# google-research/nerf-from-image

Measured on NVIDIA H100. Metric: rays_per_sec_128x128_64+64spp, higher is better.
Workload: dtype f32

## Files before the change

nerf_from_image_b200/csrc/nfi_forward_pipe.cuh:

```cuda
#pragma once
#include <type_traits>

#include "nfi_forward_tc.cuh"

namespace nfi {

#ifndef NFI_WAIT_NS
#define NFI_WAIT_NS 0
#endif
#define NFI_STEP_WAIT(bar, par) tc::mbar_wait_backoff<NFI_WAIT_NS>(bar, par)

__device__ __forceinline__ void mbar_arrive(uint64_t* bar) {
  asm volatile("mbarrier.arrive.shared::cta.b64 _, [%0];" ::"r"(tc::smem_u32(bar)) : "memory");
}

__device__ __forceinline__ float ld_relaxed(const float* p) {
  float v;
  asm volatile("ld.relaxed.cta.global.f32 %0, [%1];" : "=f"(v) : "l"(p) : "memory");
  return v;
}

__device__ __forceinline__ void column_sort(float* col, int n, int stride) {
  const int gaps[4] = {23, 10, 4, 1};
#pragma unroll 1
  for (int gi = 0; gi < 4; ++gi) {
    const int gap = gaps[gi];
    for (int i = gap; i < n; ++i) {
      const float v = col[i * stride];
      int j = i - gap;
      while (j >= 0 && col[j * stride] > v) {
        col[(j + gap) * stride] = col[j * stride];
        j -= gap;
      }
      col[(j + gap) * stride] = v;
    }
  }
}

__device__ __forceinline__ bool elect_one() {
  uint32_t pred;
  asm volatile(
      "{\n.reg .pred p;\nelect.sync _|p, 0xffffffff;\nselp.u32 %0, 1, 0, p;\n}\n"
      : "=r"(pred));
  return pred != 0;
}

struct TileCoord {
  int b, tile_x, tile_y;
};

__device__ __forceinline__ TileCoord tile_coord(int tile, int tiles_x, int tiles_y) {
  TileCoord c;
  const int per_img = tiles_x * tiles_y;
  c.b = tile / per_img;
  const int r = tile % per_img;
  const int bx = (tiles_x + 1) / 2;
  const int blk = r / 4, in = r % 4;
  int tx = 2 * (blk % bx) + (in & 1), ty = 2 * (blk / bx) + (in >> 1);
  if ((tiles_x & 1) || (tiles_y & 1)) {
    tx = r % tiles_x;
    ty = r / tiles_x;
  }
  c.tile_x = tx;
  c.tile_y = ty;
  return c;
}

constexpr int kPipeSlots = 3;
constexpr int kPipeStageBytes = 32768;
constexpr int kFwdStageBytes = 32768;
constexpr int kD2Ld = 20;
constexpr int kD2SlotBytes = kThreads * kD2Ld * 4;

__host__ __device__ inline size_t pipe_scratch_floats(int S, int nes) {
  return tc_scratch_floats_per_group(S) + (size_t)S * kThreads * nes;
}

template <int P>
struct PipeCfg {
  static constexpr int kThreadsTotal = 256 + 128 * P;
  static constexpr int kStages = P + 1;
  static constexpr int kSmA = 25600;
  static constexpr int kSmD2 = kSmA + kStages * kFwdStageBytes;
  static constexpr int kSmPal = kSmD2 + kPipeSlots * kD2SlotBytes;
  static constexpr int kSmFrac = kSmPal + 48 * 4;
  static constexpr int kSmBars = kSmFrac + 128 * 4;
  static constexpr int kNumBars = 2 * kStages + 2 * kPipeSlots + 3;
  static constexpr int kSmBytes = kSmBars + kNumBars * 8;
  static constexpr int kActRegs = 136;
  static constexpr int kShadeRegs = 80;
  static constexpr int kProducerRegs = 88;
};

constexpr float kLog2e = 1.4426950408889634f;
constexpr float kLn2 = 0.6931471805599453f;
constexpr float kPadLogit = -1e30f;

template <typename F>
__device__ __forceinline__ void decoder_step(uint64_t dsc_a, uint64_t w1_hi, uint64_t w1_lo,
                                             uint64_t w2_hi, uint64_t w2_lo,
                                             const float* __restrict__ b1, float* d2, int warp,
                                             int lane, F&& on_stage_read) {
#pragma unroll 1
  for (int mb = 0; mb < 2; ++mb) {
    float d[32];
#pragma unroll
    for (int i = 0; i < 32; ++i) d[i] = 0.f;
    tc::wgmma_fence();
    tc::layer1_mb(d, dsc_a + mb * (8192 >> 4), dsc_a + ((16384 + mb * 8192) >> 4), w1_hi, w1_lo);
    tc::wgmma_commit();
    tc::wgmma_wait<0>();
    tc::reg_fence(d);
    if (mb == 1) on_stage_read();
    uint32_t hi[8][4], lo[8][4];
    tc::softplus_frag<true>(d, b1, lane & 3, hi, lo);
    float o[8];
#pragma unroll
    for (int i = 0; i < 8; ++i) o[i] = 0.f;
    tc::wgmma_fence();
    tc::layer2_mb(o, hi, lo, w2_hi, w2_lo);
    tc::wgmma_commit();
    tc::wgmma_wait<0>();
    tc::reg_fence(o);
    tc::store_frag_rows(o, d2 + 64 * mb * kD2Ld, kD2Ld, warp, lane);
  }
}

__device__ __forceinline__ float ldcg(const float* p) {
  float v;
  asm volatile("ld.global.cg.f32 %0, [%1];" : "=f"(v) : "l"(p));
  return v;
}

template <int NOUT_PAD>
__device__ __forceinline__ void field_head_fast(const float (&out)[NOUT_PAD], const FieldConst& fc,
                                                const float* __restrict__ pal, float keep,
                                                float& sigma, float& cr, float& cg, float& cb,
                                                float* probs = nullptr) {
  constexpr int NA = NOUT_PAD - 1;
  const float d = out[0];
  if (fc.use_sdf) {
    const float nd = -d;
    const float e = tc::ex2_approx(-fabsf(nd) * (fc.inv_beta * kLog2e));
    const float sg = (nd > 0.f) ? 1.f : ((nd < 0.f) ? -1.f : 0.f);
    const float cdf = 0.5f + 0.5f * sg * (1.f - e);
    sigma = fc.inv_alpha * (cdf * keep);
  } else {
    const float x = d - 1.f;
    sigma = (x > 20.f ? x : log1pf(expf(x))) * keep;
  }
  if (fc.A > 0) {
    float m = out[1];
#pragma unroll
    for (int a = 1; a < NA; ++a) m = fmaxf(m, out[1 + a]);
    float pv[((3 * NA + 3) / 4) * 4];
#pragma unroll
    for (int i = 0; i < (3 * NA + 3) / 4; ++i) {
      const float4 t = *reinterpret_cast<const float4*>(pal + 4 * i);
      pv[4 * i] = t.x;
      pv[4 * i + 1] = t.y;
      pv[4 * i + 2] = t.z;
      pv[4 * i + 3] = t.w;
    }
    float s = 0.f, r = 0.f, g = 0.f, b = 0.f;
#pragma unroll
    for (int a = 0; a < NA; ++a) {
      const float e = tc::ex2_approx(out[1 + a] - m);
      if (probs != nullptr) probs[a] = e;
      s += e;
      r = fmaf(e, pv[3 * a + 0], r);
      g = fmaf(e, pv[3 * a + 1], g);
      b = fmaf(e, pv[3 * a + 2], b);
    }
    const float inv = __fdividef(1.f, s);
    cr = r * inv;
    cg = g * inv;
    cb = b * inv;
    if (probs != nullptr) {
#pragma unroll
      for (int a = 0; a < NA; ++a) probs[a] *= inv;
    }
  } else {
    cr = sigmoid_fast(out[1]) * 2.004f - 1.002f;
    cg = sigmoid_fast(out[2]) * 2.004f - 1.002f;
    cb = sigmoid_fast(out[3]) * 2.004f - 1.002f;
  }
}

template <int N>
struct LaneVec {
  float v[N];
};
template <int N>
__device__ __forceinline__ LaneVec<N> shift_down1(const LaneVec<N>& x, float pad, int lane) {
  LaneVec<N> y;
#pragma unroll
  for (int i = 0; i < N; ++i) {
    const float a = __shfl_down_sync(kFull, x.v[i], 1);
    const float nxt0 = (i + 1 < N) ? __shfl_sync(kFull, x.v[(i + 1 < N) ? i + 1 : i], 0) : pad;
    y.v[i] = (lane == 31) ? nxt0 : a;
  }
  return y;
}
template <int N>
__device__ __forceinline__ float pick(const LaneVec<N>& x, int idx) {
  float r = __shfl_sync(kFull, x.v[0], idx & 31);
#pragma unroll
// ... 244 lines not shown

  constexpr int kRsParts = 2 + P;
  auto rs_first = [](int part) {
    constexpr int base_rows = 32 / kRsParts, rem = 32 % kRsParts;
    return part * base_rows + min(max(part - 2, 0), rem);
  };
  auto resample_rows = [&](int part, float tnear, float tfar, size_t ray, bool valid) {
    const int first = rs_first(part), count = rs_first(part + 1) - first;
    ResampleArgs ra;
    ra.sc_w = sc_w;
    ra.sc_zf = sc_zf;
    ra.z_fine = p.z_fine;
    ra.noise_t = p.noise_t;
    ra.noise_u = p.noise_u;
    ra.frac = frac;
    ra.S = S;
    ra.wig = wig;
    ra.explicit_noise = explicit_noise;
    resample_rows_impl<NSLOT>(ra, first, count, tnear, tfar, ray, valid, lane);
  };

  if (wg >= 3) {
    asm volatile("setmaxnreg.dec.sync.aligned.u32 %0;" ::"n"(Cfg::kProducerRegs));
    const int set = wg - 3;
    uint32_t n = 0;
    uint32_t tile_it = 0;
    for (int tile = blockIdx.x; tile < n_tiles; tile += gridDim.x, ++tile_it) {
      const TileCoord tcd = tile_coord(tile, tiles_x, tiles_y);
      const int b = tcd.b;
      int px, py;
      tile_pixel(tcd.tile_x, tcd.tile_y, wig, lane, px, py);
      const bool valid = (px < p.width) && (py < p.height);
      px = min(px, p.width - 1);
      py = min(py, p.height - 1);
      const size_t ray = ((size_t)b * p.height + py) * p.width + px;
      Ray r;
      setup_ray(p, b, py, px, r);
      const float span = r.tfar - r.tnear;
      const uint32_t plane_bytes = (uint32_t)R * (uint32_t)R * 128u;
      const unsigned char* planes_b =
          reinterpret_cast<const unsigned char*>(p.planes) + (size_t)b * 3 * plane_bytes;
      for (int pass = 0; pass < (FINE ? 2 : 1); ++pass) {
        if (pass == 1) {
          tc::mbar_wait(cw_ready, tile_it & 1);
          resample_rows(2 + set, r.tnear, r.tfar, ray, valid);
          __threadfence_block();
          __syncwarp();
          if (lane == 0) mbar_arrive(zf_ready);
          tc::mbar_wait(zf_ready, tile_it & 1);
        }
        int s = (int)(((uint32_t)set + (uint32_t)P - (n % P)) % P);
        auto fetch = [&](int ss) -> float {
          if (ss >= S) return 0.f;
          if (pass == 0) return explicit_noise ? p.noise_t[ray * S + ss] : 0.f;
          return ld_relaxed(sc_zf + ss * kThreads + gt);
        };
        float nxt = fetch(s);
        for (; s < S; s += P) {
          const uint32_t st = (n + (uint32_t)s) % NS, u = (n + (uint32_t)s) / NS;
          unsigned char* const stage = base + Cfg::kSmA + st * kFwdStageBytes;
          const float cur = nxt;
          nxt = fetch(s + P);
          if (DBG && dbg_time) tprev = clock64();
          NFI_STEP_WAIT(&a_free[st], (u & 1) ^ 1);
          NFI_T(0)
          float t;
          if (pass == 0)
            t = lerp_torch(r.tnear, r.tfar, frac[s]) + cur * (span / (float)S);
          else
            t = cur;
          const float x0 = (r.ox + r.dx * t) * inv_range, x1 = (r.oy + r.dy * t) * inv_range,
                      x2 = (r.oz + r.dz * t) * inv_range;
          ByteTaps tp;
          byte_taps(x0, x1, R, 0u, tp.o[0], tp.fx[0], tp.fy[0]);
          byte_taps(x0, x2, R, plane_bytes >> 4, tp.o[1], tp.fx[1], tp.fy[1]);
          byte_taps(x1, x2, R, plane_bytes >> 3, tp.o[2], tp.fx[2], tp.fy[2]);
          NFI_T(1)
          if (dbg_window) {
            tp.o[0] &= 0x7FFu;
            tp.o[1] &= 0x7FFu;
            tp.o[2] &= 0x7FFu;
          }
          if (!dbg_skip_gather)
            gather_to_tiles_lean(planes_b, R, tp, stage, stage + 16384, 32 * wig, lane);
          NFI_T(2)
          tc::fence_async_smem();
          __syncwarp();
          if (lane == 0) mbar_arrive(&full[st]);
          NFI_T(3)
          if (DBG && dbg_time) tacc[9] += 1;
        }
        n += (uint32_t)S;
      }
    }
    if (DBG && dbg_time)
      for (int i = 0; i < 10; ++i) p.normals[i] = (float)tacc[i];
  } else if (wg == 0) {
    asm volatile("setmaxnreg.inc.sync.aligned.u32 %0;" ::"n"(Cfg::kActRegs));
    const uint32_t base_s = tc::smem_u32(base);
    const uint64_t dsc_w1_hi = tc::gmma_desc_sw128(base_s + kWiW1Hi);
    const uint64_t dsc_w1_lo = tc::gmma_desc_sw128(base_s + kWiW1Lo);
    const uint64_t dsc_w2_hi = tc::gmma_desc_sw128(base_s + kWiW2Hi);
    const uint64_t dsc_w2_lo = tc::gmma_desc_sw128(base_s + kWiW2Lo);
    const uint64_t dsc_a0 = tc::gmma_desc_sw128(base_s + Cfg::kSmA);
    uint32_t st = 0, u = 0, sl = 0, v = 0;
    auto activate = [&]() {
      if (DBG && dbg_time && tprev == 0) tprev = clock64();
      NFI_T(2)
      NFI_STEP_WAIT(&full[st], u & 1);
      NFI_STEP_WAIT(&slot_free[sl], (v & 1) ^ 1);
      NFI_T(0)
      float* d2 = d2s + sl * (kThreads * kD2Ld);
      if (!dbg_skip_consumer) {
        decoder_step(dsc_a0 + (uint64_t)st * (kFwdStageBytes >> 4), dsc_w1_hi, dsc_w1_lo, dsc_w2_hi,
                     dsc_w2_lo, b1s, d2, wig, lane, [&]() {
                       __syncwarp();
                       if (lane == 0) mbar_arrive(&a_free[st]);
                     });
      } else {
        __syncwarp();
        if (lane == 0) mbar_arrive(&a_free[st]);
      }
      __syncwarp();
      if (lane == 0) mbar_arrive(&d2_full[sl]);
      if (++st == NS) { st = 0; ++u; }
      if (++sl == kPipeSlots) { sl = 0; ++v; }
      NFI_T(1)
      if (DBG && dbg_time) tacc[9] += 1;
    };
    uint32_t tile_it = 0;
    for (int tile = blockIdx.x; tile < n_tiles; tile += gridDim.x, ++tile_it) {
      for (int s = 0; s < S; ++s) activate();
      if (FINE) {
        const TileCoord tcd = tile_coord(tile, tiles_x, tiles_y);
        int px, py;
        tile_pixel(tcd.tile_x, tcd.tile_y, wig, lane, px, py);
        const bool valid = (px < p.width) && (py < p.height);
        px = min(px, p.width - 1);
        py = min(py, p.height - 1);
        const size_t ray = ((size_t)tcd.b * p.height + py) * p.width + px;
        Ray r;
        setup_ray(p, tcd.b, py, px, r);
        tc::mbar_wait(cw_ready, tile_it & 1);
        NFI_T(3)
        resample_rows(1, r.tnear, r.tfar, ray, valid);
        __threadfence_block();
        __syncwarp();
        if (lane == 0) mbar_arrive(zf_ready);
        NFI_T(4)
        for (int s = 0; s < S; ++s) activate();
      }
    }
    if (DBG && dbg_time)
      for (int i = 0; i < 10; ++i) p.normals[16 + i] = (float)tacc[i];
  } else {
    asm volatile("setmaxnreg.dec.sync.aligned.u32 %0;" ::"n"(Cfg::kShadeRegs));
    uint32_t sl = 0, v = 0;
    FieldConst fc;
    fc.A = p.n_attention;
    fc.use_sdf = p.use_sdf;
    fc.inv_beta = p.use_sdf ? 1.f / p.beta[0] : 0.f;
    fc.inv_alpha = p.use_sdf ? 1.f / p.alpha[0] : 0.f;

    uint32_t tile_it = 0;
    for (int tile = blockIdx.x; tile < n_tiles; tile += gridDim.x, ++tile_it) {
      const TileCoord tcd = tile_coord(tile, tiles_x, tiles_y);
      const int b = tcd.b;
      int px, py;
      tile_pixel(tcd.tile_x, tcd.tile_y, wig, lane, px, py);
      const bool valid = (px < p.width) && (py < p.height);
      px = min(px, p.width - 1);
      py = min(py, p.height - 1);
      const size_t ray = ((size_t)b * p.height + py) * p.width + px;
      Ray r;
      setup_ray(p, b, py, px, r);
      const float span = r.tfar - r.tnear;

      tc::bar_sync(1, kThreads);
      if (gt < 48)
        pal[gt] = (p.n_attention > 0 && gt < p.n_attention * 3)
                      ? p.palette[(size_t)b * p.n_attention * 3 + gt]
                      : 0.f;
      tc::bar_sync(1, kThreads);
      Compositor<NE, true> comp;
      comp.init();

      auto shade = [&](float t, float& sigma, float& cr, float& cg, float& cb, float* ex) {
        const float* d2 = d2s + sl * (kThreads * kD2Ld) + gt * kD2Ld;
        if (DBG && dbg_time && tprev == 0) tprev = clock64();
        NFI_T(2)
        NFI_STEP_WAIT(&d2_full[sl], v & 1);
        NFI_T(0)
        float o16[16];
#pragma unroll
        for (int o4 = 0; o4 < 4; ++o4) {
          const float4 x = *reinterpret_cast<const float4*>(d2 + 4 * o4);
          o16[4 * o4] = x.x;
          o16[4 * o4 + 1] = x.y;
          o16[4 * o4 + 2] = x.z;
          o16[4 * o4 + 3] = x.w;
        }
// ... 176 lines not shown
```

nerf_from_image_b200/csrc/nfi_forward_tc.cuh:

```cuda
#pragma once
#include "nfi_common.cuh"
#include "nfi_forward.cuh"
#include "nfi_tc.cuh"

namespace nfi {

constexpr int kGroups = 4;
constexpr int kTcThreads = kGroups * kThreads;
constexpr int kW2Pad = 16;

constexpr int kWiW1Hi = 0;
constexpr int kWiW1Lo = 8192;
constexpr int kWiW2Hi = 16384;
constexpr int kWiW2Lo = 20480;
constexpr int kWiB1 = 24576;
constexpr int kWiB2 = kWiB1 + 256;
constexpr int kWiBytes = kWiB2 + 64;
constexpr int kSmA = 25600;
constexpr int kSmAGroup = 32768;
constexpr int kOutLd = 20;
constexpr int kSmOut = kSmA + kGroups * kSmAGroup;
constexpr int kSmPal = kSmOut + kGroups * kThreads * kOutLd * 4;
constexpr int kSmBars = kSmPal + 48 * 4;
constexpr int kSmTcBytes = kSmBars + 8;
// ... 192 lines not shown
  asm volatile("ld.global.nc.v4.f32 {%0, %1, %2, %3}, [%4];"
               : "=f"(r.x), "=f"(r.y), "=f"(r.z), "=f"(r.w)
               : "l"(p));
  return r;
}

__device__ __forceinline__ void gather_to_tiles_deep(const float* __restrict__ planes_b, int R,
                                                     const PackedTaps& tp, unsigned char* a_hi,
                                                     unsigned char* a_lo, int row0, int lane) {
  const int q = lane >> 3, k = lane & 7;
  const uint32_t plane_stride4 = (uint32_t)R * R * (kC / 4);
  const float4* base = reinterpret_cast<const float4*>(planes_b) + k;
#pragma unroll 1
  for (int g = 0; g < 8; ++g) {
    const int src = 4 * g + q;
    uint32_t off[12];
    float fx[3], fy[3];
#pragma unroll
    for (int pl = 0; pl < 3; ++pl) {
      const uint32_t o = __shfl_sync(kFull, tp.o[pl], src);
      fx[pl] = __shfl_sync(kFull, tp.fx[pl], src);
      fy[pl] = __shfl_sync(kFull, tp.fy[pl], src);
      const uint32_t o00 = (o & 0x3FFFFFFFu) * (kC / 4) + pl * plane_stride4;
      const uint32_t dx = ((o >> 30) & 1u) * (kC / 4), dy = (o >> 31) ? (uint32_t)R * (kC / 4) : 0u;
      off[4 * pl + 0] = o00;
      off[4 * pl + 1] = o00 + dx;
      off[4 * pl + 2] = o00 + dy;
      off[4 * pl + 3] = o00 + dy + dx;
    }
    float4 v[12];
#pragma unroll
    for (int i = 0; i < 12; ++i) v[i] = ldg_nc_volatile(base + off[i]);
    float2 lo = make_float2(0.f, 0.f), hi = make_float2(0.f, 0.f);
#pragma unroll
    for (int pl = 0; pl < 3; ++pl) {
      const float gx0 = 1.f - fx[pl], gy0 = 1.f - fy[pl];
      const float w[4] = {gx0 * gy0, fx[pl] * gy0, gx0 * fy[pl], fx[pl] * fy[pl]};
#pragma unroll
      for (int j = 0; j < 4; ++j) {
        const float4 x = v[4 * pl + j];
        lo = ffma2(make_float2(x.x, x.y), make_float2(w[j], w[j]), lo);
        hi = ffma2(make_float2(x.z, x.w), make_float2(w[j], w[j]), hi);
      }
    }
    const float third = 0.33333334f;
    const float4 f = make_float4(lo.x * third, lo.y * third, hi.x * third, hi.y * third);
    const float4 fh = make_float4(tc::tf32_hi(f.x), tc::tf32_hi(f.y), tc::tf32_hi(f.z),
                                  tc::tf32_hi(f.w));
    const float4 fl = make_float4(f.x - fh.x, f.y - fh.y, f.z - fh.z, f.w - fh.w);
    const uint32_t offs = tc::sw128_offset(row0 + src, k);
    *reinterpret_cast<float4*>(a_hi + offs) = fh;
    *reinterpret_cast<float4*>(a_lo + offs) = fl;
  }
}

struct ByteTaps {
  uint32_t o[3];
  float fx[3], fy[3];
};
__device__ __forceinline__ void byte_taps(float gx, float gy, int R, uint32_t plane_units,
                                          uint32_t& o, float& fx, float& fy) {
  const float m = (float)(R - 1);
  float ix = (gx + 1.f) * 0.5f * m;
  float iy = (gy + 1.f) * 0.5f * m;
  ix = fminf(m, fmaxf(ix, 0.f));
  iy = fminf(m, fmaxf(iy, 0.f));
  const float x0 = fminf(floorf(ix), m - 1.f), y0 = fminf(floorf(iy), m - 1.f);
  fx = ix - x0;
  fy = iy - y0;
  o = plane_units + (uint32_t)((int)y0 * R + (int)x0) * 8u;
}
__device__ __forceinline__ const float4* texel_ptr(const unsigned char* base, uint32_t off16) {
  uint64_t r;
  asm("mad.wide.u32 %0, %1, 16, %2;" : "=l"(r) : "r"(off16), "l"(base));
  return reinterpret_cast<const float4*>(r);
}
__device__ __forceinline__ float4 ldg_nc_volatile_next(const float4* p) {
  float4 r;
  asm volatile("ld.global.nc.v4.f32 {%0, %1, %2, %3}, [%4+128];"
               : "=f"(r.x), "=f"(r.y), "=f"(r.z), "=f"(r.w)
               : "l"(p));
  return r;
}
template <bool BF16 = false>
__device__ __forceinline__ void gather_to_tiles_lean(const unsigned char* __restrict__ planes_b,
                                                     int R, const ByteTaps& tp,
                                                     unsigned char* a_hi, unsigned char* a_lo,
                                                     int row0, int lane) {
  const int q = lane >> 3, k = lane & 7;
  const uint32_t row_units = (uint32_t)R * 8u;
#pragma unroll 1
  for (int g = 0; g < 8; ++g) {
    const int src = 4 * g + q;
    float4 v[12];
    float fx[3], fy[3];
#pragma unroll
    for (int pl = 0; pl < 3; ++pl) {
      const uint32_t o = __shfl_sync(kFull, tp.o[pl], src);
      fx[pl] = __shfl_sync(kFull, tp.fx[pl], src);
      fy[pl] = __shfl_sync(kFull, tp.fy[pl], src);
      const uint32_t a00 = o | (uint32_t)k;
      const float4* p0 = texel_ptr(planes_b, a00);
      const float4* p1 = texel_ptr(planes_b, a00 + row_units);
      v[4 * pl + 0] = ldg_nc_volatile(p0);
      v[4 * pl + 1] = ldg_nc_volatile_next(p0);
      v[4 * pl + 2] = ldg_nc_volatile(p1);
      v[4 * pl + 3] = ldg_nc_volatile_next(p1);
    }
    float2 lo = make_float2(0.f, 0.f), hi = make_float2(0.f, 0.f);
#pragma unroll
    for (int pl = 0; pl < 3; ++pl) {
      const float gx0 = 1.f - fx[pl], gy0 = 1.f - fy[pl];
      const float w[4] = {gx0 * gy0, fx[pl] * gy0, gx0 * fy[pl], fx[pl] * fy[pl]};
#pragma unroll
      for (int j = 0; j < 4; ++j) {
        const float4 x = v[4 * pl + j];
        lo = ffma2(make_float2(x.x, x.y), make_float2(w[j], w[j]), lo);
        hi = ffma2(make_float2(x.z, x.w), make_float2(w[j], w[j]), hi);
      }
    }
    const float third = 0.33333334f;
    const float4 f = make_float4(lo.x * third, lo.y * third, hi.x * third, hi.y * third);
    if constexpr (BF16) {
      uint2 h, l;
      asm("cvt.rn.bf16x2.f32 %0, %1, %2;" : "=r"(h.x) : "f"(f.y), "f"(f.x));
      asm("cvt.rn.bf16x2.f32 %0, %1, %2;" : "=r"(h.y) : "f"(f.w), "f"(f.z));
      const float rx = f.x - __uint_as_float(h.x << 16), ry = f.y - __uint_as_float(h.x & 0xFFFF0000u);
      const float rz = f.z - __uint_as_float(h.y << 16), rw = f.w - __uint_as_float(h.y & 0xFFFF0000u);
      asm("cvt.rn.bf16x2.f32 %0, %1, %2;" : "=r"(l.x) : "f"(ry), "f"(rx));
      asm("cvt.rn.bf16x2.f32 %0, %1, %2;" : "=r"(l.y) : "f"(rw), "f"(rz));
      const uint32_t offs = tc::sw64_offset(row0 + src, k >> 1) + (k & 1) * 8;
      *reinterpret_cast<uint2*>(a_hi + offs) = h;
      *reinterpret_cast<uint2*>(a_lo + offs) = l;
    } else {
      const float4 fh = make_float4(tc::tf32_hi(f.x), tc::tf32_hi(f.y), tc::tf32_hi(f.z),
                                    tc::tf32_hi(f.w));
      const float4 fl = make_float4(f.x - fh.x, f.y - fh.y, f.z - fh.z, f.w - fh.w);
      const uint32_t offs = tc::sw128_offset(row0 + src, k);
      *reinterpret_cast<float4*>(a_hi + offs) = fh;
      *reinterpret_cast<float4*>(a_lo + offs) = fl;
    }
  }
}

struct TcShared {
  unsigned char* base;
  const float* b1;
  const float* b2;
  float* pal;
  uint64_t* bars;
};

__device__ __forceinline__ TcShared tc_shared_map(unsigned char* raw) {
  TcShared s;
  s.base = raw;
  s.b1 = reinterpret_cast<const float*>(raw + kWiB1);
  s.b2 = reinterpret_cast<const float*>(raw + kWiB2);
  s.pal = reinterpret_cast<float*>(raw + kSmPal);
  s.bars = reinterpret_cast<uint64_t*>(raw + kSmBars);
  return s;
}

struct TcGroup {
  int g, gt, wig;
  unsigned char* a_hi;
  unsigned char* a_lo;
  float* out;
  uint64_t dsc_a, dsc_w1_hi, dsc_w1_lo, dsc_w2_hi, dsc_w2_lo;
};

__device__ __forceinline__ TcGroup tc_group(const TcShared& sm, int tid) {
  TcGroup q;
  q.g = __shfl_sync(kFull, tid >> 7, 0);
  q.gt = tid & 127;
  q.wig = __shfl_sync(kFull, q.gt >> 5, 0);
  q.a_hi = sm.base + kSmA + q.g * kSmAGroup;
  q.a_lo = q.a_hi + 16384;
  q.out = reinterpret_cast<float*>(sm.base + kSmOut) + q.g * kThreads * kOutLd;
  const uint32_t base_s = tc::smem_u32(sm.base);
  q.dsc_a = tc::gmma_desc_sw128(base_s + kSmA + q.g * kSmAGroup);
  q.dsc_w1_hi = tc::gmma_desc_sw128(base_s + kWiW1Hi);
  q.dsc_w1_lo = tc::gmma_desc_sw128(base_s + kWiW1Lo);
  q.dsc_w2_hi = tc::gmma_desc_sw128(base_s + kWiW2Hi);
  q.dsc_w2_lo = tc::gmma_desc_sw128(base_s + kWiW2Lo);
  return q;
}

template <int NOUT_PAD>
__device__ __forceinline__ void tile_mlp(const TcGroup& q, const TcShared& sm,
                                         float (&out)[NOUT_PAD]) {
  const int lane = q.gt & 31;
  tc::fence_async_smem();
  tc::bar_sync(1 + q.g, kThreads);
#pragma unroll 1
  for (int mb = 0; mb < 2; ++mb) {
    float d[32];
#pragma unroll
    for (int i = 0; i < 32; ++i) d[i] = 0.f;
    tc::wgmma_fence();
    tc::layer1_mb(d, q.dsc_a + mb * (8192 >> 4), q.dsc_a + ((16384 + mb * 8192) >> 4), q.dsc_w1_hi,
                  q.dsc_w1_lo);
    tc::wgmma_commit();
    tc::wgmma_wait<0>();
    tc::reg_fence(d);
    uint32_t hi[8][4], lo[8][4];
    tc::softplus_frag<false>(d, sm.b1, lane & 3, hi, lo);
// ... 283 lines not shown
```

nerf_from_image_b200/csrc/nfi_pipe.cu:

```cuda
#include <cuda_runtime.h>
#include <stdio.h>

#include "nfi_backward.cuh"
#include "nfi_backward_pipe.cuh"
#include "nfi_forward_pipe.cuh"
#include "nfi_normals_pipe.cuh"
#include "nfi_pipe_launch.h"
#include "nfi_wgrad_pipe.cuh"

namespace nfi {
namespace {

#define NFI_PCUDA(expr)                                                              \
  do {                                                                               \
    cudaError_t e__ = (expr);                                                        \
    if (e__ != cudaSuccess) {                                                        \
      snprintf(err, err_len, "%s failed: %s", #expr, cudaGetErrorString(e__));       \
      return 2;                                                                      \
    }                                                                                \
  } while (0)

template <int NP, int EX, bool FINE, bool DBG, int NSLOT>
int run_fwd(const nfi_render_params& p, const unsigned char* wimg, float* scratch, unsigned grid,
            cudaStream_t st, char* err, size_t err_len) {
  auto k = render_forward_pipe<NP, EX, FINE, 3, DBG, NSLOT>;
  NFI_PCUDA(cudaFuncSetAttribute(k, cudaFuncAttributeMaxDynamicSharedMemorySize,
                                 PipeCfg<3>::kSmBytes));
  k<<<grid, PipeCfg<3>::kThreadsTotal, PipeCfg<3>::kSmBytes, st>>>(p, wimg, scratch);
  NFI_PCUDA(cudaGetLastError());
  return 0;
}

template <int NP, int EX>
int fwd_np_ex(const nfi_render_params& p, const unsigned char* wimg, float* scratch, unsigned grid,
              cudaStream_t st, char* err, size_t err_len) {
  if constexpr (NP == 12 && EX == 0) {
    if ((p.mlp_mode & 0x1000) && p.fine_sampling)
      return run_fwd<NP, EX, true, true, 2>(p, wimg, scratch, grid, st, err, err_len);
  }
  if (p.fine_sampling && p.num_samples > 64)
    return run_fwd<NP, EX, true, false, 4>(p, wimg, scratch, grid, st, err, err_len);
  if (p.fine_sampling) return run_fwd<NP, EX, true, false, 2>(p, wimg, scratch, grid, st, err, err_len);
  return run_fwd<NP, EX, false, false, 2>(p, wimg, scratch, grid, st, err, err_len);
}

template <int NP>
int fwd_np(const nfi_render_params& p, const unsigned char* wimg, float* scratch, unsigned grid,
           cudaStream_t st, char* err, size_t err_len) {
  if (p.extra_mode == NFI_EXTRA_COORDS)
    return fwd_np_ex<NP, 1>(p, wimg, scratch, grid, st, err, err_len);
  if constexpr (NP > 4) {
    if (p.extra_mode == NFI_EXTRA_SEMANTICS)
      return fwd_np_ex<NP, 2>(p, wimg, scratch, grid, st, err, err_len);
  }
  return fwd_np_ex<NP, 0>(p, wimg, scratch, grid, st, err, err_len);
}

template <int NP, int EX, bool CAM>
int run_bwd(const nfi_render_params& p, const nfi_render_grads& g, const unsigned char* wimg,
            unsigned grid, cudaStream_t st, char* err, size_t err_len) {
  using Cfg = BwdCfg<2>;
  auto k = render_backward_pipe<NP, EX, CAM, 2>;
  NFI_PCUDA(cudaFuncSetAttribute(k, cudaFuncAttributeMaxDynamicSharedMemorySize, Cfg::kSmBytes));
  k<<<grid, Cfg::kThreadsTotal, Cfg::kSmBytes, st>>>(p, g, wimg);
  NFI_PCUDA(cudaGetLastError());
  return 0;
}

template <int NP>
int bwd_np(const nfi_render_params& p, const nfi_render_grads& g, const unsigned char* wimg,
           unsigned grid, cudaStream_t st, char* err, size_t err_len) {
  const bool cam = g.grad_origins != nullptr;
  const bool coords = p.extra_mode == NFI_EXTRA_COORDS && g.g_extra != nullptr;
  if (coords)
    return cam ? run_bwd<NP, 1, true>(p, g, wimg, grid, st, err, err_len)
               : run_bwd<NP, 1, false>(p, g, wimg, grid, st, err, err_len);
  return cam ? run_bwd<NP, 0, true>(p, g, wimg, grid, st, err, err_len)
             : run_bwd<NP, 0, false>(p, g, wimg, grid, st, err, err_len);
}

template <int NP, bool PLANES>
int run_wgrad(const nfi_render_params& p, const nfi_render_grads& g, const unsigned char* wimg,
              unsigned grid, cudaStream_t st, char* err, size_t err_len) {
  using Cfg = WgCfgT<PLANES>;
  auto k = render_wgrad_pipe<NP, PLANES>;
  NFI_PCUDA(cudaFuncSetAttribute(k, cudaFuncAttributeMaxDynamicSharedMemorySize, Cfg::kSmBytes));
  k<<<grid, Cfg::kThreadsTotal, Cfg::kSmBytes, st>>>(
      p, g, wimg, reinterpret_cast<float*>(const_cast<unsigned char*>(wimg) + 65536));
  NFI_PCUDA(cudaGetLastError());
  return 0;
}

}

size_t pipe_wgrad_workspace_bytes(unsigned grid) { return 65536 + (size_t)grid * kWgAccBytesPerCta; }

size_t pipe_scratch_bytes_per_cta(int num_samples, int nes) {
  return pipe_scratch_floats(num_samples, nes) * sizeof(float);
}

int launch_pipe_weight_image(const nfi_render_params& p, unsigned char* wimg, cudaStream_t st) {
  const int nout = 1 + (p.n_attention > 0 ? p.n_attention : 3);
  prep_weight_image<<<1, 256, 0, st>>>(p.w1, p.b1, p.w2, p.b2, nout, wimg, kLog2e,
                                       p.n_attention > 0 ? kPadLogit : 0.f,
                                       p.n_attention > 0 ? kLog2e : 1.f);
  return cudaGetLastError() == cudaSuccess ? 0 : 2;
}

int launch_pipe_forward(const nfi_render_params& p, int nout_pad, const unsigned char* wimg,
                        float* scratch, unsigned grid, cudaStream_t st, char* err,
// ... 65 lines not shown
```

nerf_from_image_b200/csrc/nfi_tc.cuh:

```cuda
#pragma once
#include <cuda_runtime.h>
#include <stdint.h>

namespace nfi {
namespace tc {

__device__ __forceinline__ uint32_t smem_u32(const void* p) {
  return static_cast<uint32_t>(__cvta_generic_to_shared(p));
}

__device__ __forceinline__ void mbar_init(uint64_t* bar, uint32_t count) {
  asm volatile("mbarrier.init.shared::cta.b64 [%0], %1;" ::"r"(smem_u32(bar)), "r"(count));
}
__device__ __forceinline__ void fence_mbar_init() {
  asm volatile("fence.mbarrier_init.release.cluster;" ::: "memory");
}
__device__ __forceinline__ bool mbar_try_wait(uint64_t* bar, uint32_t parity) {
  uint32_t ok;
  asm volatile(
      "{\n"
      ".reg .pred p;\n"
      "mbarrier.try_wait.parity.shared::cta.b64 p, [%1], %2, %3;\n"
      "selp.u32 %0, 1, 0, p;\n"
      "}\n"
// ... 160 lines not shown
      "{%0, %1, %2, %3, %4, %5, %6, %7, %8, %9, %10, %11, %12, %13, %14, %15, %16, %17, %18, %19, %20, %21, %22, %23, %24, %25, %26, %27, %28, %29, %30, %31}, %32, %33, p, 1, 1, %35, %36;\n}\n"
      : "+f"(d[0]), "+f"(d[1]), "+f"(d[2]), "+f"(d[3]), "+f"(d[4]), "+f"(d[5]), "+f"(d[6]), "+f"(d[7]), "+f"(d[8]), "+f"(d[9]), "+f"(d[10]), "+f"(d[11]), "+f"(d[12]), "+f"(d[13]), "+f"(d[14]), "+f"(d[15]), "+f"(d[16]), "+f"(d[17]), "+f"(d[18]), "+f"(d[19]), "+f"(d[20]), "+f"(d[21]), "+f"(d[22]), "+f"(d[23]), "+f"(d[24]), "+f"(d[25]), "+f"(d[26]), "+f"(d[27]), "+f"(d[28]), "+f"(d[29]), "+f"(d[30]), "+f"(d[31])
      : "l"(a), "l"(b), "r"(acc), "n"(TA), "n"(TB)
      : "memory");
}

template <int TA, int TB>
__device__ __forceinline__ void wgmma_bf16_ss_n96(float (&d)[48], uint64_t a, uint64_t b, int acc) {
  asm volatile(
      "{\n.reg .pred p;\nsetp.ne.b32 p, %50, 0;\n"
      "wgmma.mma_async.sync.aligned.m64n96k16.f32.bf16.bf16 "
      "{%0, %1, %2, %3, %4, %5, %6, %7, %8, %9, %10, %11, %12, %13, %14, %15, %16, %17, %18, %19, %20, %21, %22, %23, %24, %25, %26, %27, %28, %29, %30, %31, %32, %33, %34, %35, %36, %37, %38, %39, %40, %41, %42, %43, %44, %45, %46, %47}, %48, %49, p, 1, 1, %51, %52;\n}\n"
      : "+f"(d[0]), "+f"(d[1]), "+f"(d[2]), "+f"(d[3]), "+f"(d[4]), "+f"(d[5]), "+f"(d[6]), "+f"(d[7]), "+f"(d[8]), "+f"(d[9]), "+f"(d[10]), "+f"(d[11]), "+f"(d[12]), "+f"(d[13]), "+f"(d[14]), "+f"(d[15]), "+f"(d[16]), "+f"(d[17]), "+f"(d[18]), "+f"(d[19]), "+f"(d[20]), "+f"(d[21]), "+f"(d[22]), "+f"(d[23]), "+f"(d[24]), "+f"(d[25]), "+f"(d[26]), "+f"(d[27]), "+f"(d[28]), "+f"(d[29]), "+f"(d[30]), "+f"(d[31]), "+f"(d[32]), "+f"(d[33]), "+f"(d[34]), "+f"(d[35]), "+f"(d[36]), "+f"(d[37]), "+f"(d[38]), "+f"(d[39]), "+f"(d[40]), "+f"(d[41]), "+f"(d[42]), "+f"(d[43]), "+f"(d[44]), "+f"(d[45]), "+f"(d[46]), "+f"(d[47])
      : "l"(a), "l"(b), "r"(acc), "n"(TA), "n"(TB)
      : "memory");
}

template <int TA, int TB>
__device__ __forceinline__ void wgmma_bf16_ss_n128(float (&d)[64], uint64_t a, uint64_t b, int acc) {
  asm volatile(
      "{\n.reg .pred p;\nsetp.ne.b32 p, %66, 0;\n"
      "wgmma.mma_async.sync.aligned.m64n128k16.f32.bf16.bf16 "
      "{%0, %1, %2, %3, %4, %5, %6, %7, %8, %9, %10, %11, %12, %13, %14, %15, %16, %17, %18, %19, %20, %21, %22, %23, %24, %25, %26, %27, %28, %29, %30, %31, %32, %33, %34, %35, %36, %37, %38, %39, %40, %41, %42, %43, %44, %45, %46, %47, %48, %49, %50, %51, %52, %53, %54, %55, %56, %57, %58, %59, %60, %61, %62, %63}, %64, %65, p, 1, 1, %67, %68;\n}\n"
      : "+f"(d[0]), "+f"(d[1]), "+f"(d[2]), "+f"(d[3]), "+f"(d[4]), "+f"(d[5]), "+f"(d[6]), "+f"(d[7]), "+f"(d[8]), "+f"(d[9]), "+f"(d[10]), "+f"(d[11]), "+f"(d[12]), "+f"(d[13]), "+f"(d[14]), "+f"(d[15]), "+f"(d[16]), "+f"(d[17]), "+f"(d[18]), "+f"(d[19]), "+f"(d[20]), "+f"(d[21]), "+f"(d[22]), "+f"(d[23]), "+f"(d[24]), "+f"(d[25]), "+f"(d[26]), "+f"(d[27]), "+f"(d[28]), "+f"(d[29]), "+f"(d[30]), "+f"(d[31]), "+f"(d[32]), "+f"(d[33]), "+f"(d[34]), "+f"(d[35]), "+f"(d[36]), "+f"(d[37]), "+f"(d[38]), "+f"(d[39]), "+f"(d[40]), "+f"(d[41]), "+f"(d[42]), "+f"(d[43]), "+f"(d[44]), "+f"(d[45]), "+f"(d[46]), "+f"(d[47]), "+f"(d[48]), "+f"(d[49]), "+f"(d[50]), "+f"(d[51]), "+f"(d[52]), "+f"(d[53]), "+f"(d[54]), "+f"(d[55]), "+f"(d[56]), "+f"(d[57]), "+f"(d[58]), "+f"(d[59]), "+f"(d[60]), "+f"(d[61]), "+f"(d[62]), "+f"(d[63])
      : "l"(a), "l"(b), "r"(acc), "n"(TA), "n"(TB)
      : "memory");
}

__host__ __device__ __forceinline__ uint32_t sw128_offset(int row, int chunk) {
  return (uint32_t)((row >> 3) * 1024 + (row & 7) * 128 + ((chunk ^ (row & 7)) << 4));
}

__device__ __forceinline__ uint32_t sw64_offset(int row, int chunk) {
  return (uint32_t)(row * 64 + ((chunk ^ ((row >> 1) & 3)) << 4));
}
__device__ __forceinline__ uint32_t sw32_offset(int row, int chunk) {
  return (uint32_t)(row * 32 + ((chunk ^ ((row >> 2) & 1)) << 4));
}

__host__ __device__ __forceinline__ float tf32_hi(float x) {
#ifdef __CUDA_ARCH__
  return __uint_as_float(__float_as_uint(x) & 0xFFFFE000u);
#else
  return x;
#endif
}

__host__ __device__ constexpr int kpos_of_hidden(int j) {
  return (j & ~7) | ((j & 1) ? 4 + ((j >> 1) & 3) : ((j >> 1) & 3));
}
__host__ __device__ constexpr int afrag_slot(int e) { return ((e & 1) << 1) | (e >> 1); }

__device__ __forceinline__ void prefetch_l1(const void* p) {
  asm volatile("prefetch.global.L1 [%0];" ::"l"(p));
}

__device__ __forceinline__ float ex2_approx(float x) {
  float y;
  asm("ex2.approx.ftz.f32 %0, %1;" : "=f"(y) : "f"(x));
  return y;
}
__device__ __forceinline__ float lg2_approx(float x) {
  float y;
  asm("lg2.approx.ftz.f32 %0, %1;" : "=f"(y) : "f"(x));
  return y;
}

__device__ __forceinline__ uint32_t bf16x2_rn(float lo, float hi) {
  uint32_t y;
  asm("cvt.rn.bf16x2.f32 %0, %1, %2;" : "=r"(y) : "f"(hi), "f"(lo));
  return y;
}

__device__ __forceinline__ void layer1_mb(float (&d)[32], uint64_t a_hi, uint64_t a_lo,
                                          uint64_t w_hi, uint64_t w_lo) {
  wgmma_tf32_ss_n64(d, a_lo, w_hi, 0);
#pragma unroll
  for (int ks = 1; ks < 4; ++ks) wgmma_tf32_ss_n64(d, a_lo + 2 * ks, w_hi + 2 * ks, 1);
#pragma unroll
  for (int ks = 0; ks < 4; ++ks) wgmma_tf32_ss_n64(d, a_hi + 2 * ks, w_lo + 2 * ks, 1);
#pragma unroll
  for (int ks = 0; ks < 4; ++ks) wgmma_tf32_ss_n64(d, a_hi + 2 * ks, w_hi + 2 * ks, 1);
}
__device__ __forceinline__ void layer2_mb(float (&o)[8], const uint32_t (&hhi)[8][4],
                                          const uint32_t (&hlo)[8][4], uint64_t w2_hi,
                                          uint64_t w2_lo) {
#pragma unroll
  for (int ks = 0; ks < 8; ++ks)
    wgmma_tf32_rs_n16(o, hlo[ks], w2_hi + (ks >> 2) * 128 + (ks & 3) * 2, ks != 0);
#pragma unroll
  for (int ks = 0; ks < 8; ++ks)
    wgmma_tf32_rs_n16(o, hhi[ks], w2_lo + (ks >> 2) * 128 + (ks & 3) * 2, 1);
#pragma unroll
  for (int ks = 0; ks < 8; ++ks)
    wgmma_tf32_rs_n16(o, hhi[ks], w2_hi + (ks >> 2) * 128 + (ks & 3) * 2, 1);
}

template <int KB>
__device__ __forceinline__ void put_split(uint32_t (&hi)[KB][4], uint32_t (&lo)[KB][4], int kb,
                                          int slot, float v) {
  const float h = tf32_hi(v);
  hi[kb][slot] = __float_as_uint(h);
  lo[kb][slot] = __float_as_uint(v - h);
}

template <bool PRESCALED>
__device__ __forceinline__ float softplus_mufu(float x) {
  if (PRESCALED) {
    float l = ex2_approx(-fabsf(x));
    l = lg2_approx(l + 1.f);
    l = l + fmaxf(x, 0.f);
    return l * 0.6931471805599453f;
  }
  const float ax = fabsf(x) * -1.4426950408889634f;
  const float l = lg2_approx(1.f + ex2_approx(ax));
  return fmaf(l, 0.6931471805599453f, fmaxf(x, 0.f));
}
template <bool PRESCALED>
__device__ __forceinline__ void softplus_frag(const float (&d)[32], const float* __restrict__ b1,
                                              int t, uint32_t (&hi)[8][4], uint32_t (&lo)[8][4]) {
#pragma unroll
  for (int kb = 0; kb < 8; ++kb) {
    const float2 bb = *reinterpret_cast<const float2*>(b1 + 8 * kb + 2 * t);
#pragma unroll
    for (int e = 0; e < 4; ++e) {
      const float h = softplus_mufu<PRESCALED>(d[4 * kb + e] + ((e & 1) ? bb.y : bb.x));
      put_split(hi, lo, kb, afrag_slot(e), h);
    }
  }
}

template <int R>
__device__ __forceinline__ void store_frag_rows(const float (&d)[R], float* rows, int ld, int warp,
                                                int lane) {
  const int g = lane >> 2, t = lane & 3;
  float* r0 = rows + (16 * warp + g) * ld + 2 * t;
#pragma unroll
  for (int j = 0; j < R / 4; ++j) {
    *reinterpret_cast<float2*>(r0 + 8 * j) = make_float2(d[4 * j], d[4 * j + 1]);
    *reinterpret_cast<float2*>(r0 + 8 * ld + 8 * j) = make_float2(d[4 * j + 2], d[4 * j + 3]);
  }
}

}
}
```

nerf_from_image_b200/csrc/nfi_wgrad_pipe.cuh:

```cuda
#pragma once
#include <cuda_bf16.h>

#include "nfi_backward_pipe.cuh"

namespace nfi {

constexpr int kWgSlots = 2;
constexpr int kWgStages = 3;
constexpr int kWgFlush = 16;
constexpr size_t kWgAccBytesPerCta = 128 * 64 * sizeof(float);

template <bool PLANES>
struct WgCfgT {
  static constexpr int P = 1;
  static constexpr int kThreadsTotal = 384 + 128 * P;
  static constexpr int kStageBytes = 16384;
  static constexpr int kWbBytes = PLANES ? 32768 : 16384;
  static constexpr int kSmWb = 25600;
  static constexpr int kSmW1 = kSmWb + kWbBytes;
  static constexpr int kSmA = kSmW1 + 8192;
  static constexpr int kSmX = kSmA + kWgStages * kStageBytes;
  static constexpr int kSmE = kSmX + 65536;
  static constexpr int kSmOnes = kSmE + 8192;
  static constexpr int kSmD2 = kSmOnes + 1024;
// ... 61 lines not shown
    const __nv_bfloat16 lo = __float2bfloat16_rn(w - __bfloat162float(hi));
    const uint32_t off = tc::sw64_offset(j, c >> 3) + (c & 7) * 2;
    *reinterpret_cast<__nv_bfloat16*>(base + Cfg::kSmW1 + off) = hi;
    *reinterpret_cast<__nv_bfloat16*>(base + Cfg::kSmW1 + 4096 + off) = lo;
  }
  tc::fence_async_smem();
  if (tid == 0) {
    if (tc::smem_u32(base) & 1023u) __trap();
    for (int i = 0; i < NS; ++i) {
      tc::mbar_init(&full[i], kWarps);
      tc::mbar_init(&a_free[i], 2 * kWarps);
    }
    for (int i = 0; i < kWgSlots; ++i) {
      tc::mbar_init(&d2_full[i], kWarps);
      tc::mbar_init(&dout_ready[i], kWarps);
    }
    tc::mbar_init(d4_full, kWarps);
    tc::mbar_init(d4_free, kWarps);
    tc::mbar_init(x_ready, kWarps);
    tc::mbar_init(x_free, kWarps);
    tc::mbar_init(&wbar[0], 1);
    tc::mbar_init(&wbar[1], 1);
    tc::fence_mbar_init();
  }
  __syncthreads();
  if (tid == 0) {
    tc::mbar_expect_tx(&wbar[0], kWiBytes);
    tc::tma_bulk_g2s(base, wimg, kWiBytes, &wbar[0]);
    tc::mbar_expect_tx(&wbar[1], Cfg::kWbBytes);
    tc::tma_bulk_g2s(base + Cfg::kSmWb, wimg + 32768, Cfg::kWbBytes, &wbar[1]);
  }
  tc::mbar_wait(&wbar[0], 0);
  tc::mbar_wait(&wbar[1], 0);

  const int tiles_x = (p.width + kTileW - 1) / kTileW;
  const int tiles_y = (p.height + kTileH - 1) / kTileH;
  const int n_tiles = tiles_x * tiles_y * p.batch;
  const int my_tiles =
      ((int)blockIdx.x < n_tiles) ? (n_tiles - 1 - (int)blockIdx.x) / (int)gridDim.x + 1 : 0;
  const uint32_t total_steps = (uint32_t)my_tiles * (uint32_t)n_total;
  const int R = p.plane_res;
  const float inv_range = 1.f / p.scene_range;
  const uint32_t plane_bytes = (uint32_t)R * (uint32_t)R * 128u;

  if (wg >= 3) {
    asm volatile("setmaxnreg.dec.sync.aligned.u32 %0;" ::"n"(Cfg::kProdRegs));
    const int set = wg - 3;
    const int q = lane >> 3, kq = lane & 7;
    const uint32_t row_units = (uint32_t)R * 8u;
    uint32_t n0 = 0;
    for (int tile = blockIdx.x; tile < n_tiles; tile += gridDim.x, n0 += (uint32_t)n_total) {
      const TileCoord tcd = tile_coord(tile, tiles_x, tiles_y);
      const int b = tcd.b;
      int px, py;
      tile_pixel(tcd.tile_x, tcd.tile_y, wig, lane, px, py);
      px = min(px, p.width - 1);
      py = min(py, p.height - 1);
      const size_t ray = ((size_t)b * p.height + py) * p.width + px;
      Ray r;
      setup_ray(p, b, py, px, r);
      const unsigned char* planes_b =
          reinterpret_cast<const unsigned char*>(p.planes) + (size_t)b * 3 * plane_bytes;
      float* gplanes_b = (PLANES && g.grad_planes)
                             ? g.grad_planes + (size_t)b * 3 * (plane_bytes >> 2) : nullptr;
      MergeWalk mw;
      mw.init(p, r, ray, frac);
      int walked = 0;
      ByteTaps cur, nxt;
      auto gather_step = [&](int i, ByteTaps& tp) {
        float z = 0.f;
        while (walked <= i) {
          z = mw.pop();
          ++walked;
        }
        const float x0 = (r.ox + r.dx * z) * inv_range, x1 = (r.oy + r.dy * z) * inv_range,
                    x2 = (r.oz + r.dz * z) * inv_range;
        byte_taps(x0, x1, R, 0u, tp.o[0], tp.fx[0], tp.fy[0]);
        byte_taps(x0, x2, R, plane_bytes >> 4, tp.o[1], tp.fx[1], tp.fy[1]);
        byte_taps(x1, x2, R, plane_bytes >> 3, tp.o[2], tp.fx[2], tp.fy[2]);
        const uint32_t m = n0 + (uint32_t)i;
        const uint32_t st = m % NS, u = m / NS;
        unsigned char* const stage = base + Cfg::kSmA + st * Cfg::kStageBytes;
        NFI_STEP_WAIT(&a_free[st], (u & 1) ^ 1);
        gather_to_tiles_lean<true>(planes_b, R, tp, stage, stage + 8192, 32 * wig, lane);
        tc::fence_async_smem();
        __syncwarp();
        if (lane == 0) mbar_arrive(&full[st]);
      };
      if constexpr (!PLANES) {
        for (int i = set; i < n_total; i += P) gather_step(i, cur);
      } else {
        if (set < n_total) gather_step(set, cur);
        for (int i = set; i < n_total; i += P) {
          if (i + P < n_total) gather_step(i + P, nxt);
          const uint32_t m = n0 + (uint32_t)i;
          const float* Dw = d4s + 32 * wig * kD4Ld;
          NFI_STEP_WAIT(d4_full, m & 1);
          if (gplanes_b != nullptr) {
#pragma unroll 1
            for (int gq = 0; gq < 8; ++gq) {
              const int src = 4 * gq + q;
              const float4 d4v = *reinterpret_cast<const float4*>(Dw + src * kD4Ld + 4 * kq);
#pragma unroll
              for (int pl = 0; pl < 3; ++pl) {
                const uint32_t a00 = __shfl_sync(kFull, cur.o[pl], src) | (uint32_t)kq;
                const float fx = __shfl_sync(kFull, cur.fx[pl], src);
                const float fy = __shfl_sync(kFull, cur.fy[pl], src);
                const float gx0 = 1.f - fx, gy0 = 1.f - fy;
                const float w00 = gx0 * gy0, w01 = fx * gy0, w10 = gx0 * fy, w11 = fx * fy;
                float* gp = gplanes_b;
                red_add_v4(gp + (size_t)a00 * 4, d4v.x * w00, d4v.y * w00, d4v.z * w00, d4v.w * w00);
                red_add_v4(gp + (size_t)(a00 + 8u) * 4, d4v.x * w01, d4v.y * w01, d4v.z * w01,
                           d4v.w * w01);
                red_add_v4(gp + (size_t)(a00 + row_units) * 4, d4v.x * w10, d4v.y * w10,
                           d4v.z * w10, d4v.w * w10);
                red_add_v4(gp + (size_t)(a00 + row_units + 8u) * 4, d4v.x * w11, d4v.y * w11,
                           d4v.z * w11, d4v.w * w11);
              }
            }
          }
          __syncwarp();
          if (lane == 0) mbar_arrive(d4_free);
          cur = nxt;
        }
      }
    }
  } else if (wg == 2) {
    asm volatile("setmaxnreg.dec.sync.aligned.u32 %0;" ::"n"(Cfg::kAccRegs));
    const uint32_t base_s = tc::smem_u32(base);
    const int g4 = lane >> 2, t = lane & 3;
    float w1a[2][16], w2a[2][8], b1a[2][4];
    auto clear = [&]() {
#pragma unroll
      for (int mb = 0; mb < 2; ++mb) {
        zero(w1a[mb]);
        zero(w2a[mb]);
        zero(b1a[mb]);
      }
    };
    const int nout_w = 1 + (p.n_attention > 0 ? p.n_attention : 3);
    auto flush = [&](bool first, bool final) {
#pragma unroll
      for (int mb = 0; mb < 2; ++mb) {
#pragma unroll
        for (int half = 0; half < 2; ++half) {
          const int row = 64 * mb + 16 * wig + g4 + 8 * half, j = row & (kHid - 1);
          float* const myrow = acc_ws + ((size_t)blockIdx.x * 128 + row) * 64;
          auto put = [&](int col, float a, float b, float* gdst0, float* gdst1) {
            float2 v2 = make_float2(a, b);
            if (!first) {
              const float2 o = *reinterpret_cast<const float2*>(myrow + col);
              v2.x += o.x;
              v2.y += o.y;
            }
            if (!final) {
              *reinterpret_cast<float2*>(myrow + col) = v2;
            } else {
              if (gdst0) atomicAdd(gdst0, v2.x);
              if (gdst1) atomicAdd(gdst1, v2.y);
            }
          };
#pragma unroll
          for (int jb = 0; jb < 4; ++jb) {
            const int c = 8 * jb + 2 * t;
            put(c, w1a[mb][4 * jb + 2 * half], w1a[mb][4 * jb + 2 * half + 1],
                g.grad_w1 ? g.grad_w1 + j * kC + c : nullptr,
                g.grad_w1 ? g.grad_w1 + j * kC + c + 1 : nullptr);
// ... 400 lines not shown
```

Before: 30.03 million.

## Stage raw fp32 features and split to tf32 pairs in consumer registers

```diff
diff --git a/nerf_from_image_b200/csrc/nfi_forward_pipe.cuh b/nerf_from_image_b200/csrc/nfi_forward_pipe.cuh
--- a/nerf_from_image_b200/csrc/nfi_forward_pipe.cuh
+++ b/nerf_from_image_b200/csrc/nfi_forward_pipe.cuh
@@ -68,7 +68,7 @@
 
 constexpr int kPipeSlots = 3;
 constexpr int kPipeStageBytes = 32768;
-constexpr int kFwdStageBytes = 32768;
+constexpr int kFwdStageBytes = 16384;
 constexpr int kD2Ld = 20;
 constexpr int kD2SlotBytes = kThreads * kD2Ld * 4;
 
@@ -96,6 +96,22 @@
 constexpr float kLn2 = 0.6931471805599453f;
 constexpr float kPadLogit = -1e30f;
 
+__device__ __forceinline__ void decoder_layer2(const float (&d)[32], uint64_t w2_hi, uint64_t w2_lo,
+                                               const float* __restrict__ b1, float* d2, int warp,
+                                               int lane) {
+  uint32_t hi[8][4], lo[8][4];
+  tc::softplus_frag<true>(d, b1, lane & 3, hi, lo);
+  float o[8];
+#pragma unroll
+  for (int i = 0; i < 8; ++i) o[i] = 0.f;
+  tc::wgmma_fence();
+  tc::layer2_mb(o, hi, lo, w2_hi, w2_lo);
+  tc::wgmma_commit();
+  tc::wgmma_wait<0>();
+  tc::reg_fence(o);
+  tc::store_frag_rows(o, d2, kD2Ld, warp, lane);
+}
+
 template <typename F>
 __device__ __forceinline__ void decoder_step(uint64_t dsc_a, uint64_t w1_hi, uint64_t w1_lo,
                                              uint64_t w2_hi, uint64_t w2_lo,
@@ -112,17 +128,39 @@
     tc::wgmma_wait<0>();
     tc::reg_fence(d);
     if (mb == 1) on_stage_read();
-    uint32_t hi[8][4], lo[8][4];
-    tc::softplus_frag<true>(d, b1, lane & 3, hi, lo);
-    float o[8];
-#pragma unroll
-    for (int i = 0; i < 8; ++i) o[i] = 0.f;
+    decoder_layer2(d, w2_hi, w2_lo, b1, d2 + 64 * mb * kD2Ld, warp, lane);
+  }
+}
+
+template <typename F>
+__device__ __forceinline__ void decoder_step_fp32(const unsigned char* stage, uint64_t w1_hi,
+                                                  uint64_t w1_lo, uint64_t w2_hi, uint64_t w2_lo,
+                                                  const float* __restrict__ b1, float* d2, int warp,
+                                                  int lane, F&& on_stage_read) {
+  float fa[4][4], fb[4][4];
+  tc::load_afrag_sw128(fa, stage, 0, warp, lane);
+  tc::load_afrag_sw128(fb, stage, 64, warp, lane);
+  on_stage_read();
+#pragma unroll 1
+  for (int mb = 0; mb < 2; ++mb) {
+    uint32_t a_hi[4][4], a_lo[4][4];
+#pragma unroll
+    for (int kb = 0; kb < 4; ++kb)
+#pragma unroll
+      for (int s = 0; s < 4; ++s) tc::put_split(a_hi, a_lo, kb, s, fa[kb][s]);
+    float d[32];
+#pragma unroll
+    for (int i = 0; i < 32; ++i) d[i] = 0.f;
     tc::wgmma_fence();
-    tc::layer2_mb(o, hi, lo, w2_hi, w2_lo);
+    tc::layer1_mb_rs(d, a_hi, a_lo, w1_hi, w1_lo);
     tc::wgmma_commit();
     tc::wgmma_wait<0>();
-    tc::reg_fence(o);
-    tc::store_frag_rows(o, d2 + 64 * mb * kD2Ld, kD2Ld, warp, lane);
+    tc::reg_fence(d);
+    decoder_layer2(d, w2_hi, w2_lo, b1, d2 + 64 * mb * kD2Ld, warp, lane);
+#pragma unroll
+    for (int kb = 0; kb < 4; ++kb)
+#pragma unroll
+      for (int s = 0; s < 4; ++s) fa[kb][s] = fb[kb][s];
   }
 }
 
@@ -533,9 +571,8 @@
             tp.o[2] &= 0x7FFu;
           }
           if (!dbg_skip_gather)
-            gather_to_tiles_lean(planes_b, R, tp, stage, stage + 16384, 32 * wig, lane);
+            gather_to_tiles_lean<TileStore::kFp32>(planes_b, R, tp, stage, nullptr, 32 * wig, lane);
           NFI_T(2)
-          tc::fence_async_smem();
           __syncwarp();
           if (lane == 0) mbar_arrive(&full[st]);
           NFI_T(3)
@@ -553,7 +590,6 @@
     const uint64_t dsc_w1_lo = tc::gmma_desc_sw128(base_s + kWiW1Lo);
     const uint64_t dsc_w2_hi = tc::gmma_desc_sw128(base_s + kWiW2Hi);
     const uint64_t dsc_w2_lo = tc::gmma_desc_sw128(base_s + kWiW2Lo);
-    const uint64_t dsc_a0 = tc::gmma_desc_sw128(base_s + Cfg::kSmA);
     uint32_t st = 0, u = 0, sl = 0, v = 0;
     auto activate = [&]() {
       if (DBG && dbg_time && tprev == 0) tprev = clock64();
@@ -563,11 +599,11 @@
       NFI_T(0)
       float* d2 = d2s + sl * (kThreads * kD2Ld);
       if (!dbg_skip_consumer) {
-        decoder_step(dsc_a0 + (uint64_t)st * (kFwdStageBytes >> 4), dsc_w1_hi, dsc_w1_lo, dsc_w2_hi,
-                     dsc_w2_lo, b1s, d2, wig, lane, [&]() {
-                       __syncwarp();
-                       if (lane == 0) mbar_arrive(&a_free[st]);
-                     });
+        decoder_step_fp32(base + Cfg::kSmA + st * kFwdStageBytes, dsc_w1_hi, dsc_w1_lo, dsc_w2_hi,
+                          dsc_w2_lo, b1s, d2, wig, lane, [&]() {
+                            __syncwarp();
+                            if (lane == 0) mbar_arrive(&a_free[st]);
+                          });
       } else {
         __syncwarp();
         if (lane == 0) mbar_arrive(&a_free[st]);
diff --git a/nerf_from_image_b200/csrc/nfi_forward_tc.cuh b/nerf_from_image_b200/csrc/nfi_forward_tc.cuh
--- a/nerf_from_image_b200/csrc/nfi_forward_tc.cuh
+++ b/nerf_from_image_b200/csrc/nfi_forward_tc.cuh
@@ -298,7 +298,8 @@
                : "l"(p));
   return r;
 }
-template <bool BF16 = false>
+enum class TileStore { kTf32Pair, kBf16Pair, kFp32 };
+template <TileStore MODE = TileStore::kTf32Pair>
 __device__ __forceinline__ void gather_to_tiles_lean(const unsigned char* __restrict__ planes_b,
                                                      int R, const ByteTaps& tp,
                                                      unsigned char* a_hi, unsigned char* a_lo,
@@ -337,7 +338,9 @@
     }
     const float third = 0.33333334f;
     const float4 f = make_float4(lo.x * third, lo.y * third, hi.x * third, hi.y * third);
-    if constexpr (BF16) {
+    if constexpr (MODE == TileStore::kFp32) {
+      *reinterpret_cast<float4*>(a_hi + tc::sw128_offset(row0 + src, k)) = f;
+    } else if constexpr (MODE == TileStore::kBf16Pair) {
       uint2 h, l;
       asm("cvt.rn.bf16x2.f32 %0, %1, %2;" : "=r"(h.x) : "f"(f.y), "f"(f.x));
       asm("cvt.rn.bf16x2.f32 %0, %1, %2;" : "=r"(h.y) : "f"(f.w), "f"(f.z));
diff --git a/nerf_from_image_b200/csrc/nfi_pipe.cu b/nerf_from_image_b200/csrc/nfi_pipe.cu
--- a/nerf_from_image_b200/csrc/nfi_pipe.cu
+++ b/nerf_from_image_b200/csrc/nfi_pipe.cu
@@ -20,12 +20,20 @@
     }                                                                                \
   } while (0)
 
+constexpr int kSmemPerSm = 228 * 1024, kSmemReservedPerCta = 1024;
+static_assert(PipeCfg<3>::kSmBytes + kSmemReservedPerCta <= 132 * 1024,
+              "render_forward_pipe no longer fits the 132 KiB carve-out step");
+constexpr int kFwdCarveoutPct =
+    ((PipeCfg<3>::kSmBytes + kSmemReservedPerCta) * 100 + kSmemPerSm - 1) / kSmemPerSm;
+
 template <int NP, int EX, bool FINE, bool DBG, int NSLOT>
 int run_fwd(const nfi_render_params& p, const unsigned char* wimg, float* scratch, unsigned grid,
             cudaStream_t st, char* err, size_t err_len) {
   auto k = render_forward_pipe<NP, EX, FINE, 3, DBG, NSLOT>;
   NFI_PCUDA(cudaFuncSetAttribute(k, cudaFuncAttributeMaxDynamicSharedMemorySize,
                                  PipeCfg<3>::kSmBytes));
+  NFI_PCUDA(cudaFuncSetAttribute(k, cudaFuncAttributePreferredSharedMemoryCarveout,
+                                 kFwdCarveoutPct));
   k<<<grid, PipeCfg<3>::kThreadsTotal, PipeCfg<3>::kSmBytes, st>>>(p, wimg, scratch);
   NFI_PCUDA(cudaGetLastError());
   return 0;
diff --git a/nerf_from_image_b200/csrc/nfi_tc.cuh b/nerf_from_image_b200/csrc/nfi_tc.cuh
--- a/nerf_from_image_b200/csrc/nfi_tc.cuh
+++ b/nerf_from_image_b200/csrc/nfi_tc.cuh
@@ -266,6 +266,30 @@
 #pragma unroll
   for (int ks = 0; ks < 4; ++ks) wgmma_tf32_ss_n64(d, a_hi + 2 * ks, w_hi + 2 * ks, 1);
 }
+__device__ __forceinline__ void layer1_mb_rs(float (&d)[32], const uint32_t (&a_hi)[4][4],
+                                             const uint32_t (&a_lo)[4][4], uint64_t w_hi,
+                                             uint64_t w_lo) {
+  wgmma_tf32_rs_n64(d, a_lo[0], w_hi, 0);
+#pragma unroll
+  for (int ks = 1; ks < 4; ++ks) wgmma_tf32_rs_n64(d, a_lo[ks], w_hi + 2 * ks, 1);
+#pragma unroll
+  for (int ks = 0; ks < 4; ++ks) wgmma_tf32_rs_n64(d, a_hi[ks], w_lo + 2 * ks, 1);
+#pragma unroll
+  for (int ks = 0; ks < 4; ++ks) wgmma_tf32_rs_n64(d, a_hi[ks], w_hi + 2 * ks, 1);
+}
+__device__ __forceinline__ void load_afrag_sw128(float (&f)[4][4], const unsigned char* tile,
+                                                 int row0, int warp, int lane) {
+  const int g = lane >> 2, t = lane & 3;
+  const int r = row0 + 16 * warp + g;
+#pragma unroll
+  for (int kb = 0; kb < 4; ++kb) {
+#pragma unroll
+    for (int s = 0; s < 4; ++s) {
+      const int row = r + 8 * (s & 1), chunk = 2 * kb + (s >> 1);
+      f[kb][s] = *reinterpret_cast<const float*>(tile + sw128_offset(row, chunk) + 4 * t);
+    }
+  }
+}
 __device__ __forceinline__ void layer2_mb(float (&o)[8], const uint32_t (&hhi)[8][4],
                                           const uint32_t (&hlo)[8][4], uint64_t w2_hi,
                                           uint64_t w2_lo) {
diff --git a/nerf_from_image_b200/csrc/nfi_wgrad_pipe.cuh b/nerf_from_image_b200/csrc/nfi_wgrad_pipe.cuh
--- a/nerf_from_image_b200/csrc/nfi_wgrad_pipe.cuh
+++ b/nerf_from_image_b200/csrc/nfi_wgrad_pipe.cuh
@@ -167,7 +167,7 @@
         const uint32_t st = m % NS, u = m / NS;
         unsigned char* const stage = base + Cfg::kSmA + st * Cfg::kStageBytes;
         NFI_STEP_WAIT(&a_free[st], (u & 1) ^ 1);
-        gather_to_tiles_lean<true>(planes_b, R, tp, stage, stage + 8192, 32 * wig, lane);
+        gather_to_tiles_lean<TileStore::kBf16Pair>(planes_b, R, tp, stage, stage + 8192, 32 * wig, lane);
         tc::fence_async_smem();
         __syncwarp();
         if (lane == 0) mbar_arrive(&full[st]);
```

Result: faster. 31.70 million, median of 6 (+5.6%).
